# torognes/vsearch

Hardware: AMD Instinct MI355X
Metric: GCUPS (useful DP cells/s of the search16 global-alignment path: DP + traceback + CIGAR) (higher is better)
Workload: dtype int16

## Files before the change

vsearch_amd/csrc/vsx_device.hip:

```cpp
#include <hip/hip_runtime.h>
#include <type_traits>
#include <cstdlib>
#include <atomic>
#include "vsx_internal.h"

typedef unsigned int u32;
typedef unsigned int u32x4 __attribute__((ext_vector_type(4)));
typedef unsigned int u32x3 __attribute__((ext_vector_type(3)));
typedef short s2 __attribute__((ext_vector_type(2)));
typedef unsigned short us2 __attribute__((ext_vector_type(2)));

#define DEV __device__ __forceinline__
struct __attribute__((aligned(4))) Pair2 { unsigned int x, y; };

#define SIGN2 0x80008000u

DEV s2 S2(u32 x) { return __builtin_bit_cast(s2, x); }
DEV us2 U2(u32 x) { return __builtin_bit_cast(us2, x); }
DEV u32 UI(s2 x) { return __builtin_bit_cast(u32, x); }
DEV u32 UI(us2 x) { return __builtin_bit_cast(u32, x); }

DEV u32 sadd(u32 a, u32 b) { return UI(__builtin_elementwise_add_sat(S2(a), S2(b))); }
DEV u32 ssub(u32 a, u32 b) { return UI(__builtin_elementwise_sub_sat(S2(a), S2(b))); }
DEV u32 pmax(u32 a, u32 b) { return UI(__builtin_elementwise_max(S2(a), S2(b))); }
// ... 911 lines not shown
              u32 cv = vin((u32) (uint16_t) P.hleft[ii < 0 ? 0 : ii]);
              if (TOPPAD && L == 0 && xs < pad) cv = vin((u32) (uint16_t) (((xs == pad - 1) ? 0 : -P.top_open) + (xs - pad - 1) * tl));
              tbL[64 + tid] = cv;
            }
        }
      else if (L == 0)
        {
#pragma unroll
          for (int cc = 0; cc < 17; ++cc)
            {
              int c = c0 - 1 + cc;
              if (c > jj) c = jj;
              const u32 corner = (u32) (uint16_t) (((TOPPAD && pad > 0) ? -P.top_open : 0) - (pad + 2) * tl);
              tbL[(cc + 1) * 64 + tid] = (c < 0) ? vin(corner) : vin((u32) (uint16_t) (P.htop[c] - pad * tl));
            }
        }
      else
        {
          const int Lp = L - 1;
          const int sp = Lp >> 4, lp = Lp & 15;
          stage_top(rowck + (size_t) VSX_CK_SLOT(CK8, g, lp) * (CK8 ? 3 : 4), VSX_ROWCK_PAIR_DW(CK8), (long) ((size_t) sp * steps) + (long) (c0 - 1 + lp),
                    (long) (rowsteps >> 1) - 1);
          if (c0 == 0) tbL[64 + tid] = vin((u32) (uint16_t) P.hleft[i0 - 1]);
        }
      stage_symbols(c0);

      u32 hp[RT], ee[RT], qa[RT];
      const u32 qrq_i = pen_pk(P.qrq_i_pk);
      const u32 rq_i = pen_pk(P.rq_i_pk);
      const bool lastrow_here = lastpos && (!MID || hh == 1);
      const u32 qrq_last = lastrow_here ? pen_pk(P.qrq_r_pk) : qrq_i;
      const u32 rq_last = lastrow_here ? pen_pk(P.rq_r_pk) : rq_i;
      if (m == 0)
        {
#pragma unroll
          for (int x = 0; x < RT; ++x)
            {
              int ii = i0 + r0h + x; if (ii > Q - 1) ii = Q - 1;
              if (ii < 0) ii = 0;
              const u32 hl = vin((u32) (uint16_t) P.hleft[ii]);
              hp[x] = hl;
              ee[x] = A::sub(hl, (ii < Q - 1) ? qrq_i : pen_pk(P.qrq_r_pk));
            }
          if (TOPPAD && L == 0 && pad > 0)
            {
#pragma unroll
              for (int x = 0; x < RT; ++x)
                if (r0h + x < pad)
                  {
                    const int xs = r0h + x;
                    const int sh = (xs - pad - 1) * tl;
                    hp[x] = vin((u32) (uint16_t) (((xs == pad - 1) ? 0 : -P.top_open) + sh));
                    ee[x] = A::sub(vin((u32) (uint16_t) (-P.top_open - P.top_step + sh)), qrq_i);
                  }
            }
        }
      else
        {
          if (CK8)
            {
              constexpr int NBQ = MID ? VSX_COLCK_NBH(RT) : VSX_COLCK_NB(R, true);
              Quad fq[NBQ];
              if (MID)
                {
                  const u32 * cb = colck + ((size_t) s * nblk + (size_t) (m - 1)) * COL_DW + VSX_COLCK_CDW(VSX_COLCK_NB(R, true), VSX_CK_SLOT(true, g, l), 0)
                                   + (size_t) (hh * NBQ) * (4 * VSX_COLCK_CG);
#pragma unroll
                  for (int b = 0; b < NBQ; ++b) fq[b] = *reinterpret_cast<const Quad *>(cb + (size_t) b * (4 * VSX_COLCK_CG));
                }
              else
                {
                  const u32 * cb = colck + ((size_t) s * nblk + (size_t) (m - 1)) * COL_DW + VSX_COLCK_CDW(VSX_COLCK_NB(R, true), VSX_CK_SLOT(true, g, l), 0);
#pragma unroll
                  for (int b = 0; b < NBQ; ++b) fq[b] = *reinterpret_cast<const Quad *>(cb + (size_t) b * (4 * VSX_COLCK_CG));
                }
              auto flat = [&](int z) -> u32 {
                const Quad & qd = fq[z >> 2];
                return (z & 3) == 0 ? qd.x : (z & 3) == 1 ? qd.y : (z & 3) == 2 ? qd.z : qd.w;
              };
#pragma unroll
              for (int x = 0; x < RT; ++x)
                {
                  const u32 h = half_lo(flat(x), hi) & 0xffffu;
                  const u32 dd = flat(RT + (x >> 1)) >> (8 * ((x & 1) * 2 + (hi ? 1 : 0)));
                  hp[x] = h;
                  ee[x] = h - (u32) (int) (int8_t) (dd & 0xffu);
                }
            }
          else if (R % 2 == 0)
            {
              const u32 * cb = colck + ((size_t) s * nblk + (size_t) (m - 1)) * COL_DW + VSX_COLCK_DW(R, g * 16 + l, 0);
              constexpr int NBQ = (2 * R) / 4 ? (2 * R) / 4 : 1;
              Quad fq[NBQ];
#pragma unroll
              for (int b = 0; b < NBQ; ++b) fq[b] = *reinterpret_cast<const Quad *>(cb + (size_t) b * (4 * VSX_COLCK_G));
              auto flat = [&](int z) -> u32 {
                const Quad & qd = fq[z >> 2];
                return (z & 3) == 0 ? qd.x : (z & 3) == 1 ? qd.y : (z & 3) == 2 ? qd.z : qd.w;
              };
#pragma unroll
              for (int x = 0; x < R; ++x) { hp[x] = inck(half_lo(flat(x), hi)); ee[x] = inck(half_lo(flat(R + x), hi)); }
            }
          else
            {
#pragma unroll
              for (int x = 0; x < R; ++x)
                {
                  hp[x] = inck(half_lo(colck_at(s, m - 1, g * 16 + l, x), hi));
                  ee[x] = inck(half_lo(colck_at(s, m - 1, g * 16 + l, R + x), hi));
                }
            }
        }
      {
        u32 w[(RT + 3) / 4];
#pragma unroll
        for (int e = 0; e < (RT + 3) / 4; ++e) w[e] = *reinterpret_cast<const u32_unaligned *>(q + i0 + r0h + 4 * e);
#pragma unroll
        for (int x = 0; x < RT; ++x)
          qa[x] = (w[x >> 2] >> (8 * (x & 3))) & 15u;
        if (TOPPAD && L == 0)
          {
#pragma unroll
            for (int x = 0; x < RT; ++x)
              if (r0h + x < pad) qa[x] = 16u;
          }
      }
      u32 diag = tbL[64 + tid] & 0xffffu;

      const bool tile_int = CK8 && RT > 1 && RT <= 16 && !__any(busy && (c0 + cmax >= D - 1));
      const bool top_is_border = (L == 0) && (hh == 0);
      for (int cc = 0; cc <= cmax; ++cc)
        {
          const int c = c0 + cc;
          const u32 qrt = (c < D - 1) ? qrt_i16 : qrt_r16;
          const u32 rt = (c < D - 1) ? rt_i16 : rt_r16;
          const u32 tbv = tbL[(cc + 2) * 64 + tid];
          const u32 topH = tbv & 0xffffu;
          u32 F = top_is_border ? A::sub(topH, qrt) : (tbv >> 16);
          const u32 b16 = (((u32) symL[(cc >> 1) * 64 + tid] >> (4 * (cc & 1))) & 15u) * 32u;
          u32 Hd = diag;
          u32 acc = 0;
          auto row = [&](int x, auto int_tag) __attribute__((always_inline)) {
            constexpr bool INT = decltype(int_tag)::value;
            const u32 V = A::score((int16_t) Ssh[b16 + qa[x]]);
            const u32 h0 = A::add(Hd, V);
            const u32 dU = A::dif(h0, F);
            const u32 h1 = A::max(h0, F);
            const u32 dL = A::dif(h1, ee[x]);
            const u32 h2 = A::max(h1, ee[x]);
            Hd = hp[x];
            hp[x] = h2;
            const bool plain = INT && x < RT - 1;
            const u32 qrq = (x == RT - 1) ? qrq_last : qrq_i;
            const u32 rq = (x == RT - 1) ? rq_last : rq_i;
            const u32 hf = A::sub(h2, qrt);
            const u32 f = INT ? F : A::sub(F, rt);
            const u32 dEU = A::dif(hf, f);
            F = A::max(f, hf);
            const u32 he = plain ? hf : A::sub(h2, qrq);
            const u32 e = plain ? ee[x] : A::sub(ee[x], rq);
            const u32 dEL = A::dif(he, e);
            ee[x] = A::max(e, he);
            acc = A::fun(A::fun(A::fun(A::fun(acc, dU), dL), dEU), dEL);
          };
          if (one_row)
            {
              row(0, std::false_type {});
              bitsL[(cc * ND) * 64 + tid] = (uint16_t) A::one_row_word(acc);
            }
          else
            {
#pragma unroll
              for (int x4 = 0; x4 < RT; x4 += 4)
                if (x4 <= rmax)
                  {
                    if (tile_int)
                      {
#pragma unroll
                        for (int y = 0; y < 4; ++y)
                          if (x4 + y < RT) row(x4 + y, std::true_type {});
                      }
                    else
                      {
#pragma unroll
                        for (int y = 0; y < 4; ++y)
                          if (x4 + y < RT) row(x4 + y, std::false_type {});
                      }
                    bitsL[(cc * ND + (x4 >> 2)) * 64 + tid] = (uint16_t) acc;
                  }
            }
          diag = topH;
        }

      if (busy)
        {
          while (r >= r0h && j >= c0 && (!TOPPAD || i >= 0))
            {
              const int cw = j - c0;
              const int rv = r - r0h;
              const u32 w = bitsL[(cw * ND + (rv >> 2)) * 64 + tid];
              int rid = RT - 4 * (rv >> 2);
              if (rid > 4) rid = 4;
              const u32 bts = A::nibble(w, rid, rv & 3);
              ++al;
              if (op == 1 && (bts & A::EXT_LEFT)) { --j; push(1); }
              else if (op == 2 && (bts & A::EXT_UP)) { --i; --r; push(2); }
              else if (bts & A::LEFT) { if (op != 1) ++ga; --j; push(1); }
              else if (bts & A::UP) { if (op != 2) ++ga; --i; --r; push(2); }
              else { --i; --r; --j; push(0); }
#if VSX_TB_STATS
              atomicAdd(&vsx_tb_stats_dev[3], 1ull);
#endif
            }
          if (r < 0 && L > 0) { --L; r = (L == 0 ? rtop0 : R) - 1; }
        }
    }
#if VSX_TB_STATS
  if (valid) atomicAdd(&vsx_tb_stats_dev[5], 1ull);
#endif
  if (!valid) return;

  VsxPairOut o;
  o.pad = 0; o.nruns = 0; o.run_off = 0;
  if (so.overflow)
    {
      o.score = 32767; o.aligned = 0; o.matches = 0; o.mismatches = 0; o.gaps = 0;
      out[pair_ids[k]] = o;
      rank_note(FL, pair_ids[k], 0u, 32767, 0.0);
      return;
    }
  if (i >= 0) { al += (u32) (i + 1); if (op != 2) ++ga; push_n(2, (u32) (i + 1)); }
  if (j >= 0) { al += (u32) (j + 1); if (op != 1) ++ga; push_n(1, (u32) (j + 1)); }
  if (op >= 0) my[nruns++] = (runlen << 2) | (u32) op;

  u32 ma = 0, mi = 0;
  {
    int qi = Q - 1, tj = D - 1;
    for (u32 x = 0; x < nruns; ++x)
      {
        const u32 w = my[x];
        const int len = (int) (w >> 2);
        const u32 o2 = w & 3u;
        if (o2 == 0)
          {
            for (int b = 0; b < len; b += 8)
              {
                const int rem = (len - b < 8) ? len - b : 8;
                const unsigned long long aw = *reinterpret_cast<const u64_unaligned *>(q + (qi - b - 7));
                const unsigned long long cw = *reinterpret_cast<const u64_unaligned *>(d + (tj - b - 7));
                const unsigned long long ones = 0x0101010101010101ull;
                const unsigned long long x = aw & cw;
                unsigned long long t = (x | (x >> 1) | (x >> 2) | (x >> 3)) & ones;
                if (P.n_mismatch)
                  {
                    const unsigned long long a15 = aw & (aw >> 1) & (aw >> 2) & (aw >> 3);
                    const unsigned long long c15 = cw & (cw >> 1) & (cw >> 2) & (cw >> 3);
                    t &= ~(a15 | c15);
                  }
                t &= ~0ull << (8 * (8 - rem));
                const u32 m8 = (u32) __builtin_popcountll(t);
                ma += m8;
                mi += (u32) rem - m8;
              }
            qi -= len; tj -= len;
          }
        else if (o2 == 1) tj -= len;
        else qi -= len;
      }
  }

  u32 verdict = 0;
  double idv = 0.0;
  if (FL.enabled && nruns > 0) verdict = accept_verdict(FL, Q, D, (int) al, (int) ma, (int) mi, (int) ga, my[nruns - 1], my[0], &idv);
  if (verdict == 3u) nruns = 0;
  rank_note(FL, pair_ids[k], verdict, (int) so.score, idv);

  const unsigned long long base = atomicAdd(cursor, (unsigned long long) nruns);
  if (base + nruns <= runs_capacity)
    for (u32 x = 0; x < nruns; ++x) runs[base + x] = my[x];

  o.score = so.score;
  o.aligned = (uint16_t) al; o.matches = (uint16_t) ma; o.mismatches = (uint16_t) mi; o.gaps = (uint16_t) ga;
  o.pad = (uint16_t) verdict;
  o.nruns = nruns;
  o.run_off = base;
  out[pair_ids[k]] = o;
}


DEV u32 pk_add(u32 a, u32 b) { return UI((us2) (U2(a) + U2(b))); }
DEV u32 pk_sub(u32 a, u32 b) { return psubw(a, b); }
#ifdef VSX_TB2_WAVES_N
#define VSX_TB2_WAVES(R_, MID_) VSX_TB2_WAVES_N
#endif
#ifndef VSX_TB2_WAVES
#define VSX_TB2_WAVES(R_, MID_) 3
#endif
#ifndef VSX_TB_LDSSTAGE
#define VSX_TB_LDSSTAGE 1
#endif
#ifndef VSX_TB_LDSSTAGE_FOR
#define VSX_TB_LDSSTAGE_FOR(R_) ((R_) == 14 || (R_) == 16 || (R_) >= 26)
#endif
template <int R, bool MID>
__global__ void __launch_bounds__(64) __attribute__((amdgpu_waves_per_eu(VSX_TB2_WAVES(R, MID), 8)))
vsx_traceback_tilt_kernel(const VsxDevParams P, const VsxFilterDev FL, const VsxTask * __restrict__ tasks,
                          const u32 * __restrict__ pair_slot, const u32 * __restrict__ pair_ids, u32 npairs,
                          const uint8_t * __restrict__ qc, const uint8_t * __restrict__ tc,
                          const u32 * __restrict__ ck, const VsxSlotOut * __restrict__ slot,
                          u32 * __restrict__ slab, const uint64_t * __restrict__ slab_off,
                          u32 * __restrict__ runs, uint64_t runs_capacity, unsigned long long * cursor,
                          VsxPairOut * __restrict__ out)
{
  static_assert(R >= 4 && (!MID || R % 2 == 0), "R = 1 keeps the first kernel");
  constexpr int RT = MID ? R / 2 : R;
  constexpr int HR = (RT + 1) / 2;
  constexpr int NG = (HR + 3) / 4;
  constexpr int XL = RT - 1 - HR;
  constexpr int NBQ = MID ? VSX_COLCK_NBH(RT) : VSX_COLCK_NB(R, true);
  __shared__ uint8_t Ssh[512];
  __shared__ u32 Ssh4[16];
  constexpr int BITS_DW = 17 * NG * 64, SYM_DW = 10 * 64 / 4;
  __shared__ __attribute__((aligned(16))) u32 arenaL[BITS_DW + SYM_DW + 19 * 64];
  u32 * const bitsL = arenaL;
  uint8_t * const symL = reinterpret_cast<uint8_t *>(arenaL + BITS_DW);
  u32 * const tbL = arenaL + BITS_DW + SYM_DW;
  constexpr bool LSTAGE = (VSX_TB_LDSSTAGE != 0) && VSX_TB_LDSSTAGE_FOR(R) && (BITS_DW + SYM_DW >= 9 * 64 * 4);
  const int tid = (int) threadIdx.x;
  for (int x = tid; x < 512; x += 64)
    Ssh[x] = (uint8_t) (((x & 31) < 16) ? P.matrix[(x >> 5) * 16 + (x & 15)] : (int16_t) (-P.top_step + 2 * P.tilt));
  if (tid < 16)
    {
      const int16_t * mr = P.matrix + tid * 16;
      Ssh4[tid] = (u32) (uint8_t) mr[1] | ((u32) (uint8_t) mr[2] << 8) | ((u32) (uint8_t) mr[4] << 16) | ((u32) (uint8_t) mr[8] << 24);
    }
  __syncthreads();

  const u32 k = blockIdx.x * 64 + (u32) threadIdx.x;
  const bool valid = k < npairs;
  const u32 ts = pair_slot[valid ? k : 0];
  const u32 task = ts >> 3, sl = ts & 7;
  const VsxTask & T = tasks[task];
  const VsxSlotOut so = slot[ts];
  const bool live = valid && !so.overflow;

  const int Q = (int) T.qlen;
  const int D = (int) T.tlen[sl];
  const u32 steps32 = T.steps;
  const unsigned long long dir_off = T.dir_off;
  constexpr size_t COL_DW = (size_t) 64 * 4 * VSX_COLCK_NB(R, true);
  const int g = (int) (sl >> 1) + (int) T.group0;
  const bool hi = (sl & 1) != 0;
  const u32 half_sel = hi ? 0x07060302u : 0x05040100u;
  const u32 bias = P.max3 ? 0x3E00u : 0x8000u;
  const u32 bias_pk = bias * 0x10001u;
  const int tl = P.tilt;
  auto pk16 = [](int v) -> u32 { const u32 x = (u32) v & 0xffffu; return x | (x << 16); };
  auto pk2 = [](int lo, int hi_) -> u32 { return ((u32) lo & 0xffffu) | ((u32) hi_ << 16); };
  const int qrt_i = P.qrt_i, qrt_r = P.qrt_r, rt_i = P.rt_i, rt_r = P.rt_r;
  const int qrq_i = (int) (int16_t) (P.qrq_i_pk & 0xffffu), rq_i = (int) (int16_t) (P.rq_i_pk & 0xffffu);
  const int qrq_r = (int) (int16_t) (P.qrq_r_pk & 0xffffu), rq_r = (int) (int16_t) (P.rq_r_pk & 0xffffu);
  const uint8_t * __restrict__ q = qc + T.qoff;
  const uint8_t * __restrict__ d = tc + T.toff[sl];
  u32 * __restrict__ my = slab + slab_off[valid ? k : 0];

  int i = live ? Q - 1 : -1, j = live ? D - 1 : -1;
  int L = (Q + R - 1) / R - 1;
  int r = R - 1;
  int op = -1;
  u32 runlen = 0, nruns = 0;
  u32 al = 0, ga = 0;
  auto push_n = [&](int newop, u32 n) {
    if (newop == op) { runlen += n; return; }
    if (op >= 0) my[nruns++] = (runlen << 2) | (u32) op;
    op = newop;
    runlen = n;
  };
  auto push = [&](int newop) { push_n(newop, 1u); };

  if (live)
    {
      const int lv = (so.leave == 0xFFFFu) ? -1 : (int) so.leave;
      if (lv < D - 1)
        {
          const u32 n = (u32) (D - 1 - lv);
          al += n; ++ga;
          push_n(1, n);
          j = lv;
        }
    }

  const u32 mA[4] = {0x01010101u, 0x02020202u, 0x04040404u, 0x08080808u};
  const u32 mB[4] = {0x10101010u, 0x20202020u, 0x40404040u, 0x80808080u};

#if VSX_TB_STATS
  const unsigned long long t_kernel0 = __builtin_readcyclecounter();
  unsigned n_iter = 0;
  unsigned long long tphase[6] = {0, 0, 0, 0, 0, 0};
#endif
  for (;;)
    {
      const bool busy = (i >= 0) && (j >= 0);
      if (!__any(busy)) break;
#if VSX_TB_STATS
      ++n_iter;
#endif

      u32 Qb = (u32) Q, stb = steps32;
      unsigned long long dob = dir_off;
      asm volatile("" : "+v"(Qb), "+v"(stb), "+v"(dob));
      const int total_lanes = ((int) Qb + R - 1) / R;
      const int rcnt0 = (int) Qb - (total_lanes - 1) * R;
      const int pad = R - rcnt0;
      const int nstrips = (total_lanes + 15) >> 4;
      const size_t steps = stb;
      const size_t nblk = (steps + 15) >> 4;
      const size_t rowsteps = ((size_t) nstrips * steps + 1) & ~(size_t) 1;
      const size_t rowck_dw = (rowsteps >> 1) * VSX_ROWCK_PAIR_DW(true);
      const u32 * __restrict__ rowck = ck + dob;
      const u32 * __restrict__ colck = rowck + rowck_dw;
      const u32 * __restrict__ midck = colck + (size_t) nstrips * nblk * COL_DW;
      const int s = L >> 4, l = L & 15;
      const int jj = busy ? j : 0;
      const int m = (jj + l) >> 4;
      const int c0 = (16 * m - l) > 0 ? 16 * m - l : 0;
      const int c0b = (m >= 1 && 16 * (m - 1) - l > 0) ? 16 * (m - 1) - l : 0;
      const int i0 = (L == 0) ? -pad : rcnt0 + (L - 1) * R;
      const bool lastpos = (L == total_lanes - 1);
      const int hh = (MID && busy && r >= RT) ? 1 : 0;
      const int r0h = hh * RT;
      const bool lastrow_here = lastpos && (!MID || hh == 1);
      const bool top_is_border = (L == 0) && (hh == 0);
#if VSX_TB_STATS & 1
      {
        const unsigned key = busy ? (((unsigned) task & 0x3FFu) << 22) | ((unsigned) L << 12) | ((unsigned) m << 1) | (unsigned) hh : 0xFFFFFFFFu;
        bool leader = busy;
        for (int o = 1; o < 8; ++o)
          {
            const unsigned other = (unsigned) __shfl((int) key, (tid & ~7) | ((tid - o) & 7), 64);
            if ((tid & 7) >= o && other == key) leader = false;
          }
        const unsigned long long nb = __popcll(__ballot(busy)), nl = __popcll(__ballot(leader));
        if (tid == 0) { atomicAdd(&vsx_tb_stats_dev[1], nb); atomicAdd(&vsx_tb_stats_dev[2], nl); }
      }
#endif

      struct TileIn { Trio v3[LSTAGE ? 1 : 9]; int par; Quad fq[NBQ]; u32 sw[5]; };
      auto load_tile = [&](TileIn & in, const int cst, const int mleft) __attribute__((always_inline)) {
        in.par = 0;
        if (!top_is_border)
          {
            const u32 * base;
            long gstart;
            if (MID && hh == 1)
              {
                base = midck + (size_t) VSX_CK_SLOT(true, g, l) * 3;
                gstart = (long) ((size_t) s * steps) + (long) (cst - 1 + l);
              }
            else
              {
                const int Lp = L - 1, sp = Lp >> 4, lp = Lp & 15;
                base = rowck + (size_t) VSX_CK_SLOT(true, g, lp) * 3;
                gstart = (long) ((size_t) sp * steps) + (long) (cst - 1 + lp);
              }
            const long p0 = gstart >> 1;
            in.par = (int) (gstart - 2 * p0);
            const u32 * bp = base + p0 * (long) VSX_ROWCK_PAIR_DW(true);
            if (LSTAGE)
              {
#pragma unroll
                for (int e = 0; e < 9; ++e)
                  __builtin_amdgcn_global_load_lds((const __attribute__((address_space(1))) void *) (bp + e * VSX_ROWCK_PAIR_DW(true)),
                                                   (__attribute__((address_space(3))) void *) (arenaL + e * 256), 12, 0, 0);
              }
            else
              {
#pragma unroll
            for (int e = 0; e < 9; ++e) in.v3[LSTAGE ? 0 : e] = *reinterpret_cast<const Trio *>(bp + e * VSX_ROWCK_PAIR_DW(true));
              }
          }
        const u32 * cb = colck + ((size_t) s * nblk + (size_t) (mleft > 0 ? mleft : 0)) * COL_DW + VSX_COLCK_CDW(VSX_COLCK_NB(R, true), VSX_CK_SLOT(true, g, l), 0)
                         + (MID ? (size_t) (hh * NBQ) * (4 * VSX_COLCK_CG) : 0);
#pragma unroll
        for (int b = 0; b < NBQ; ++b) in.fq[b] = *reinterpret_cast<const Quad *>(cb + (size_t) b * (4 * VSX_COLCK_CG));
#pragma unroll
        for (int e = 0; e < 5; ++e) in.sw[e] = *reinterpret_cast<const u32_unaligned *>(d + cst + 4 * e);
      };

      u32 qcd[HR], qsel[HR];
      bool plain_acgt = true;
      {
        u32 w[(RT + 3) / 4];
#pragma unroll
        for (int e = 0; e < (RT + 3) / 4; ++e) w[e] = *reinterpret_cast<const u32_unaligned *>(q + i0 + r0h + 4 * e);
        auto code_of = [&](int x) -> u32 {
          const int xx = x < RT ? x : RT - 1;
          u32 c = (w[xx >> 2] >> (8 * (xx & 3))) & 15u;
          if (L == 0 && r0h + xx < pad) c = 16u;
          return c;
        };
#pragma unroll
        for (int x = 0; x < HR; ++x)
          {
            const u32 a = code_of(x), b = code_of(x + HR);
            qcd[x] = a | (b << 16);
            const u32 ia = (a >> 1) - (a >> 3), ib = (b >> 1) - (b >> 3);
            qsel[x] = ia | 0x0C000C00u | ((4u + ib) << 16);
            plain_acgt = plain_acgt && (a == 1 || a == 2 || a == 4 || a == 8) && (b == 1 || b == 2 || b == 4 || b == 8);
          }
      }
      const bool fastV = !__any(busy && !plain_acgt);

      const u32 qrq_pk_i = pk16(qrq_i), rq_pk_i = pk16(rq_i);
      const u32 qrq_pk_x = pk2(qrq_i, lastrow_here ? qrq_r : qrq_i), rq_pk_x = pk2(rq_i, lastrow_here ? rq_r : rq_i);

      auto recompute = [&](const TileIn & in, const bool border_left, const int cst, const int rmax_raw, const int cmax, const bool tile_int)
                       __attribute__((always_inline)) {
        if (top_is_border)
          {
            const u32 corner = (u32) (uint16_t) (((pad > 0) ? -P.top_open : 0) - (pad + 2) * tl);
#pragma unroll
            for (int e = 0; e < 17; ++e)
              {
                int c = cst - 1 + e;
                if (c > jj) c = jj;
                tbL[e * 64 + tid] = (c < 0) ? (corner & 0xffffu) : (u32) (uint16_t) (P.htop[c] - pad * tl);
              }
          }
        else
          {
            u32 * dst = tbL + tid - in.par * 64;
            if (LSTAGE) asm volatile("s_waitcnt vmcnt(0)" ::: "memory");
#pragma unroll
            for (int e = 0; e < 9; ++e)
              {
                Trio raw;
                if (LSTAGE) raw = *reinterpret_cast<const Trio *>(arenaL + e * 256 + tid * 4);
                else raw = in.v3[LSTAGE ? 0 : e];
                const u32 h0 = (half_lo(raw.x, hi) - bias) & 0xffffu, h1 = (half_lo(raw.y, hi) - bias) & 0xffffu;
                const u32 dd = hi ? (raw.z >> 8) : raw.z;
                const int d0 = (int) (int8_t) (dd & 0xffu), d1 = (int) (int8_t) ((dd >> 16) & 0xffu);
                if (e > 0 || in.par == 0) dst[(2 * e) * 64] = h0 | ((h0 - (u32) d0) << 16);
                dst[(2 * e + 1) * 64] = h1 | ((h1 - (u32) d1) << 16);
              }
            if (cst == 0)
              {
                u32 cv;
                if (MID && hh == 1)
                  {
                    const int xs = RT - 1;
                    int ii = i0 + xs; if (ii > Q - 1) ii = Q - 1;
                    cv = (u32) (uint16_t) P.hleft[ii < 0 ? 0 : ii];
                    if (L == 0 && xs < pad) cv = (u32) (uint16_t) (((xs == pad - 1) ? 0 : -P.top_open) + (xs - pad - 1) * tl);
                  }
                else cv = (u32) (uint16_t) P.hleft[i0 - 1];
                tbL[tid] = cv;
              }
          }
#pragma unroll
        for (int c2 = 0; c2 < 10; ++c2)
          {
            const u32 lo = (in.sw[c2 >> 1] >> (16 * (c2 & 1))) & 15u, hi4 = (in.sw[c2 >> 1] >> (16 * (c2 & 1) + 8)) & 15u;
            symL[c2 * 64 + tid] = (uint8_t) (lo | (hi4 << 4));
          }
        u32 hp[HR], ee[HR];
        if (border_left)
          {
#pragma unroll
            for (int x = 0; x < HR; ++x)
              {
                u32 hv[2], ev[2];
#pragma unroll
                for (int hf_ = 0; hf_ < 2; ++hf_)
                  {
                    const int xs = r0h + x + hf_ * HR;
                    int ii = i0 + xs; if (ii > Q - 1) ii = Q - 1;
                    if (ii < 0) ii = 0;
                    asm volatile("" : "+v"(ii));
                    int hl = P.hleft[ii];
                    int e0 = hl - ((ii < Q - 1) ? qrq_i : qrq_r);
                    if (L == 0 && xs < pad)
                      {
                        const int sh = (xs - pad - 1) * tl;
                        hl = ((xs == pad - 1) ? 0 : -P.top_open) + sh;
                        e0 = -P.top_open - P.top_step + sh - qrq_i;
                      }
                    hv[hf_] = (u32) hl & 0xffffu; ev[hf_] = (u32) e0 & 0xffffu;
                  }
                hp[x] = hv[0] | (hv[1] << 16);
                ee[x] = ev[0] | (ev[1] << 16);
              }
          }
        else
          {
            auto flat = [&](int z) -> u32 {
              const Quad & qd = in.fq[z >> 2];
              return (z & 3) == 0 ? qd.x : (z & 3) == 1 ? qd.y : (z & 3) == 2 ? qd.z : qd.w;
            };
#pragma unroll
            for (int x = 0; x < HR; ++x)
              {
                const int xa = x, xb = (x + HR < RT) ? x + HR : RT - 1;
                const u32 h = pk_sub(__builtin_amdgcn_perm(flat(xb), flat(xa), half_sel), bias_pk);
                const int da = (int) (int8_t) ((flat(RT + (xa >> 1)) >> (8 * ((xa & 1) * 2 + (hi ? 1 : 0)))) & 0xffu);
                const int db = (int) (int8_t) ((flat(RT + (xb >> 1)) >> (8 * ((xb & 1) * 2 + (hi ? 1 : 0)))) & 0xffu);
                hp[x] = h;
                ee[x] = pk_sub(h, ((u32) da & 0xffffu) | ((u32) db << 16));
              }
          }
        const int xmax = rmax_raw >= HR ? HR - 1 : rmax_raw;
        u32 tb_prev = tbL[tid];
        u32 Hd_end = 0, F_end = 0;
        u32 cr_prev = 0, qrt_prev = 0, rt_prev = 0;
        auto sym_at = [&](int it) -> u32 { return ((u32) symL[(it >> 1) * 64 + tid] >> (4 * (it & 1))) & 15u; };
        const bool FASTV_any = fastV;
        u32 tbv_n = tbL[64 + tid];
        u32 cr_n = FASTV_any ? Ssh4[sym_at(0)] : sym_at(0) * 32u;
        u32 sy_n = sym_at(1);
        auto column = [&](const int it, auto int_tag, auto fast_tag, auto first_tag) __attribute__((always_inline)) {
          constexpr bool INT = decltype(int_tag)::value;
          constexpr bool FASTV = decltype(fast_tag)::value;
          constexpr bool FIRST = decltype(first_tag)::value;
          const int c = cst + it;
          const u32 tbv = tbv_n;
          const u32 cr = cr_n;
          cr_n = FASTV ? Ssh4[sy_n] : sy_n * 32u;
          tbv_n = tbL[(it + 2) * 64 + tid];
          sy_n = sym_at(it + 2);
          u32 qrt_pk = 0, rt_pk = 0;
          if (!INT)
            {
              const u32 ql = (u32) ((c < D - 1) ? qrt_i : qrt_r) & 0xffffu, rl = (u32) ((c < D - 1) ? rt_i : rt_r) & 0xffffu;
              qrt_pk = ql | (qrt_prev << 16); rt_pk = rl | (rt_prev << 16);
              qrt_prev = ql; rt_prev = rl;
            }
          else qrt_pk = pk16(qrt_i);
          u32 Hd = __builtin_amdgcn_perm(Hd_end, tb_prev, 0x05040100u);
          u32 F = __builtin_amdgcn_perm(F_end, tbv, 0x05040302u);
          if (top_is_border)
            F = __builtin_amdgcn_perm(F_end, ((tbv & 0xffffu) - (INT ? (u32) qrt_i : (qrt_pk & 0xffffu))), 0x05040100u);
#pragma unroll
          for (int g4 = 0; g4 < NG; ++g4)
            if (4 * g4 <= xmax)
              {
                u32 acc = 0;
#pragma unroll
                for (int x = 4 * g4; x < 4 * g4 + 4; ++x)
                  if (x < HR)
                    {
                      u32 V;
                      if (FASTV) V = __builtin_amdgcn_perm(cr_prev, cr, qsel[x]);
                      else
                        {
                          u32 qc2 = qcd[x];
                          asm volatile("" : "+v"(qc2));
                          V = (u32) Ssh[cr + (qc2 & 0xffffu)] | ((u32) Ssh[cr_prev + (qc2 >> 16)] << 16);
                        }
                      const u32 h0 = pk_add(Hd, V);
                      const u32 dU = ssub(h0, F);
                      const u32 h1 = pmax(h0, F);
                      const u32 dL = ssub(h1, ee[x]);
                      const u32 h2 = pmax(h1, ee[x]);
                      Hd = hp[x];
                      hp[x] = FIRST ? bfi(0x0000FFFFu, h2, hp[x]) : h2;
                      const u32 hf = pk_sub(h2, qrt_pk);
                      const u32 f = INT ? F : pk_sub(F, rt_pk);
                      const u32 dEU = ssub(hf, f);
                      F = pmax(f, hf);
                      const bool plain = INT && x != XL;
                      const u32 he = plain ? hf : pk_sub(h2, x == XL ? qrq_pk_x : qrq_pk_i);
                      const u32 e = plain ? ee[x] : pk_sub(ee[x], x == XL ? rq_pk_x : rq_pk_i);
                      const u32 dEL = ssub(he, e);
                      const u32 en = pmax(e, he);
                      ee[x] = FIRST ? bfi(0x0000FFFFu, en, ee[x]) : en;
                      acc = a_bfi(mA[x & 3], __builtin_amdgcn_perm(dL, dU, 0x0B0A0908u), acc);
                      acc = a_bfi(mB[x & 3], __builtin_amdgcn_perm(dEL, dEU, 0x0B0A0908u), acc);
                    }
                bitsL[(it * NG + g4) * 64 + tid] = acc;
              }
          Hd_end = Hd;
          F_end = F;
          tb_prev = tbv;
          cr_prev = cr;
        };
        auto sweep = [&](auto int_tag, auto fast_tag) __attribute__((always_inline)) {
          column(0, int_tag, fast_tag, std::true_type {});
          for (int it = 1; it <= cmax + 1; ++it) column(it, int_tag, fast_tag, std::false_type {});
        };
        if (tile_int) { if (fastV) sweep(std::true_type {}, std::true_type {}); else sweep(std::true_type {}, std::false_type {}); }
        else          { if (fastV) sweep(std::false_type {}, std::true_type {}); else sweep(std::false_type {}, std::false_type {}); }
      };
      auto walk = [&](const int cst) __attribute__((always_inline)) {
        while (r >= r0h && j >= cst && i >= 0)
          {
            const int cw = j - cst;
            const int rv = r - r0h;
            const bool up_half = rv >= HR;
            const int rx = up_half ? rv - HR : rv;
            const u32 w = bitsL[((cw + (up_half ? 1 : 0)) * NG + (rx >> 2)) * 64 + tid] >> ((rx & 3) + (up_half ? 8 : 0));
            ++al;
            const u32 inI = (op == 1) ? 1u : 0u, inD = (op == 2) ? 1u : 0u;
            const u32 c1 = inI & (w >> 20);
            const u32 c2 = (c1 ^ 1u) & inD & (w >> 4);
            const u32 c12 = c1 | c2;
            const u32 c3 = (c12 ^ 1u) & (w >> 16);
            const u32 c4 = ((c12 | c3) ^ 1u) & w;
            const u32 isI = (c1 | c3) & 1u, isD = (c2 | c4) & 1u;
            const int newop = (int) (isI + 2u * isD);
            ga += ((c3 & (inI ^ 1u)) | (c4 & (inD ^ 1u))) & 1u;
            j -= (int) (isD ^ 1u);
            const int di = (int) (isI ^ 1u);
            i -= di; r -= di;
            if (newop != op)
              {
                if (op >= 0) my[nruns++] = (runlen << 2) | (u32) op;
                op = newop;
                runlen = 0;
              }
            ++runlen;
#if VSX_TB_STATS & 1
            atomicAdd(&vsx_tb_stats_dev[3], 1ull);
#endif
          }
      };

#if VSX_TB_STATS & 2
#define TBMARK(k_) do { __builtin_amdgcn_s_waitcnt(0); const unsigned long long now_ = __builtin_readcyclecounter(); tphase[k_] += now_ - tmark; tmark = now_; } while (0)
      unsigned long long tmark = __builtin_readcyclecounter();
#else
#define TBMARK(k_) do { } while (0)
#endif
#pragma unroll 1
      for (int tno = 0; tno < 2; ++tno)
        {
          const bool need = (tno == 0) ? busy : (busy && (m >= 1) && (r >= r0h) && (i >= 0) && (j >= 0) && (j < c0));
          if (tno == 1 && !__any(need)) break;
          const int cst = tno ? c0b : c0;
          TileIn in;
          load_tile(in, cst, tno ? m - 2 : m - 1);
          TBMARK(3 * tno);
          const int rmax_raw = __builtin_amdgcn_readfirstlane(wave_max_i32(need ? r - r0h : 0));
          const int cmax = __builtin_amdgcn_readfirstlane(wave_max_i32(need ? j - cst : 0));
          const bool tile_int = tno ? true : !__any(busy && (c0 + cmax >= D - 1));
          recompute(in, tno ? (m <= 1) : (m == 0), cst, rmax_raw, cmax, tile_int);
          TBMARK(3 * tno + 1);
          if (need) walk(cst);
          TBMARK(3 * tno + 2);
        }
      if (busy && r < 0 && L > 0) { --L; r = R - 1; }
    }
#if VSX_TB_STATS
  if (valid) atomicAdd(&vsx_tb_stats_dev[5], 1ull);
  if (tid == 0)
    {
      atomicAdd(&vsx_tb_stats_dev[15], __builtin_readcyclecounter() - t_kernel0); atomicAdd(&vsx_tb_stats_dev[0], (unsigned long long) n_iter);
      for (int k2 = 0; k2 < 6; ++k2) atomicAdd(&vsx_tb_stats_dev[8 + k2], tphase[k2]);
    }
#endif
  if (!valid) return;

  VsxPairOut o;
  o.pad = 0; o.nruns = 0; o.run_off = 0;
  if (so.overflow)
    {
      o.score = 32767; o.aligned = 0; o.matches = 0; o.mismatches = 0; o.gaps = 0;
      out[pair_ids[k]] = o;
      rank_note(FL, pair_ids[k], 0u, 32767, 0.0);
      return;
    }
  if (i >= 0) { al += (u32) (i + 1); if (op != 2) ++ga; push_n(2, (u32) (i + 1)); }
  if (j >= 0) { al += (u32) (j + 1); if (op != 1) ++ga; push_n(1, (u32) (j + 1)); }
  if (op >= 0) my[nruns++] = (runlen << 2) | (u32) op;

  u32 ma = 0, mi = 0;
  {
    int qi = Q - 1, tj = D - 1;
    for (u32 x = 0; x < nruns; ++x)
      {
        const u32 w = my[x];
        const int len = (int) (w >> 2);
        const u32 o2 = w & 3u;
        if (o2 == 0)
          {
            for (int b = 0; b < len; b += 8)
              {
                const int rem = (len - b < 8) ? len - b : 8;
                const unsigned long long aw = *reinterpret_cast<const u64_unaligned *>(q + (qi - b - 7));
                const unsigned long long cw = *reinterpret_cast<const u64_unaligned *>(d + (tj - b - 7));
                const unsigned long long ones = 0x0101010101010101ull;
                const unsigned long long x2 = aw & cw;
                unsigned long long t = (x2 | (x2 >> 1) | (x2 >> 2) | (x2 >> 3)) & ones;
                if (P.n_mismatch)
                  {
                    const unsigned long long a15 = aw & (aw >> 1) & (aw >> 2) & (aw >> 3);
                    const unsigned long long c15 = cw & (cw >> 1) & (cw >> 2) & (cw >> 3);
                    t &= ~(a15 | c15);
                  }
                t &= ~0ull << (8 * (8 - rem));
                const u32 m8 = (u32) __builtin_popcountll(t);
                ma += m8;
                mi += (u32) rem - m8;
              }
            qi -= len; tj -= len;
          }
        else if (o2 == 1) tj -= len;
        else qi -= len;
      }
  }

  u32 verdict = 0;
  double idv = 0.0;
  if (FL.enabled && nruns > 0) verdict = accept_verdict(FL, Q, D, (int) al, (int) ma, (int) mi, (int) ga, my[nruns - 1], my[0], &idv);
  if (verdict == 3u) nruns = 0;
  rank_note(FL, pair_ids[k], verdict, (int) so.score, idv);

  const unsigned long long base = atomicAdd(cursor, (unsigned long long) nruns);
  if (base + nruns <= runs_capacity)
    for (u32 x = 0; x < nruns; ++x) runs[base + x] = my[x];

  o.score = so.score;
  o.aligned = (uint16_t) al; o.matches = (uint16_t) ma; o.mismatches = (uint16_t) mi; o.gaps = (uint16_t) ga;
  o.pad = (uint16_t) verdict;
  o.nruns = nruns;
  o.run_off = base;
  out[pair_ids[k]] = o;
}

DEV u32 map4(u32 ch)
{
  const u32 c = ch | 0x20u;
  if (((ch | 0x20u) < 'a') || ((ch | 0x20u) > 'z') || ((ch & 0xC0u) != 0x40u)) return 0;
  switch (c)
    {
    case 'a': return 1;  case 'b': return 14; case 'c': return 2;  case 'd': return 13;
    case 'g': return 4;  case 'h': return 11; case 'k': return 12; case 'm': return 3;
    case 'n': return 15; case 'r': return 5;  case 's': return 6;  case 't': return 8;
    case 'u': return 8;  case 'v': return 7;  case 'w': return 9;  case 'y': return 10;
    default: return 0;
    }
}

__global__ void __launch_bounds__(256)
vsx_encode_kernel(const uint8_t * __restrict__ ascii, uint8_t * __restrict__ codes, uint64_t nbytes)
{
  __shared__ uint8_t lut[256];
  lut[threadIdx.x] = (uint8_t) map4(threadIdx.x);
  __syncthreads();
  const uint64_t nvec = nbytes >> 4;
  const uint64_t stride = (uint64_t) gridDim.x * blockDim.x;
  for (uint64_t v = (uint64_t) blockIdx.x * blockDim.x + threadIdx.x; v < nvec; v += stride)
    {
      const uint4 in = reinterpret_cast<const uint4 *>(ascii)[v];
      u32 w[4] = {in.x, in.y, in.z, in.w};
      u32 o[4];
#pragma unroll
      for (int x = 0; x < 4; ++x)
        o[x] = (u32) lut[w[x] & 0xff] | ((u32) lut[(w[x] >> 8) & 0xff] << 8) |
               ((u32) lut[(w[x] >> 16) & 0xff] << 16) | ((u32) lut[w[x] >> 24] << 24);
      reinterpret_cast<uint4 *>(codes)[v] = make_uint4(o[0], o[1], o[2], o[3]);
    }
  if (blockIdx.x == 0 && threadIdx.x < (nbytes & 15))
    {
      const uint64_t p = (nvec << 4) + threadIdx.x;
      codes[p] = lut[ascii[p]];
    }
}

__global__ void __launch_bounds__(256)
vsx_purity_kernel(const uint8_t * __restrict__ codes, const uint64_t * __restrict__ off,
                  const uint32_t * __restrict__ len, uint64_t nseq, uint8_t * __restrict__ impure)
{
  const uint64_t s = (uint64_t) blockIdx.x * 4 + (threadIdx.x >> 6);
  if (s >= nseq) return;
  const int lane = threadIdx.x & 63;
  const uint8_t * p = codes + off[s];
  const uint32_t n = len[s];
  int bad = 0;
  for (uint32_t x = lane; x < n; x += 64)
    {
      const u32 c = p[x];
      bad |= !((c != 0) && ((c & (c - 1)) == 0));
    }
  const unsigned long long any = __ballot(bad);
  if (lane == 0) impure[s] = any ? 1 : 0;
}

__global__ void __launch_bounds__(256)
vsx_max3_selftest_kernel(u32 * bad)
{
  const u32 x = blockIdx.x * 256u + threadIdx.x;
  if (x > 0x7BFFu) return;
  const u32 edge[8] = {0u, 1u, 0x03FFu, 0x0400u, 0x3C00u, 0x3E00u, 0x7BFEu, 0x7BFFu};
  u32 wrong = 0;
  for (u32 k = 0; k < 64; ++k)
    {
      const u32 h = (x * 2654435761u) ^ (k * 0x9E3779B9u);
      const u32 y = (k < 8) ? edge[k] : (h >> 7) % 0x7C00u;
      const u32 z = (k < 16) ? edge[(k + 3) & 7] : (h >> 17) % 0x7C00u;
      const u32 a = x | (y << 16), b = y | (z << 16), c = z | (x << 16);
      const u32 got = pk_max3_bits(a, b, c);
      const u32 m = x > y ? (x > z ? x : z) : (y > z ? y : z);
      if (got != (m | (m << 16))) ++wrong;
      const u32 pa = h ^ (x << 13), pb = (h * 0x85EBCA6Bu) ^ k;
      const u32 pg = __builtin_amdgcn_perm(pa, pb, 0x0B0A0908u);
      const u32 pe = ((pb >> 15) & 1u) * 0xFFu | (((pb >> 31) & 1u) * 0xFFu) << 8 | (((pa >> 15) & 1u) * 0xFFu) << 16 | (((pa >> 31) & 1u) * 0xFFu) << 24;
      if (pg != pe) atomicAdd(bad + 1, 1u);
    }
  if (wrong) atomicAdd(bad, wrong);
}
static std::atomic<int> g_tb_v1_dev[65];
extern "C" void vsx_internal_set_tb_v2(int device, int on) { g_tb_v1_dev[device < 0 || device > 64 ? 64 : device].store(on ? 0 : 1); }
extern "C" hipError_t vsx_launch_max3_selftest(u32 * d_bad, hipStream_t st)
{
  hipLaunchKernelGGL(vsx_max3_selftest_kernel, dim3((0x7C00 + 255) / 256), dim3(256), 0, st, d_bad);
  return hipGetLastError();
}

static const int kRows[] = {1, 4, 8, 10, 12, 14, 16, 18, 20, 22, 24, 26, 28, 32};

extern "C" const int * vsx_supported_rows(int * count)
{
  *count = (int) (sizeof(kRows) / sizeof(kRows[0]));
  return kRows;
}

extern "C" hipError_t vsx_launch_encode(const uint8_t * d_ascii, uint8_t * d_codes, uint64_t nbytes, hipStream_t st)
{
  if (nbytes == 0) return hipSuccess;
  uint64_t blocks = ((nbytes >> 4) + 255) / 256;
  if (blocks < 1) blocks = 1;
  if (blocks > 256 * 8) blocks = 256 * 8;
  hipLaunchKernelGGL(vsx_encode_kernel, dim3((unsigned) blocks), dim3(256), 0, st, d_ascii, d_codes, nbytes);
  return hipGetLastError();
}

extern "C" hipError_t vsx_launch_purity(const uint8_t * d_codes, const uint64_t * d_off, const uint32_t * d_len,
                                        uint64_t nseq, uint8_t * d_impure, hipStream_t st)
{
  if (nseq == 0) return hipSuccess;
  hipLaunchKernelGGL(vsx_purity_kernel, dim3((unsigned) ((nseq + 3) / 4)), dim3(256), 0, st,
                     d_codes, d_off, d_len, nseq, d_impure);
  return hipGetLastError();
}

#define VSX_FWD_GO(GRID_, ...) hipLaunchKernelGGL((vsx_forward_kernel<__VA_ARGS__>), dim3(GRID_), dim3(64), 0, st, P, d_tasks, q, t, dir, strip, slot, ntasks)
#define VSX_FWD_GO4(GRID_, ...) hipLaunchKernelGGL((vsx_forward_kernel<__VA_ARGS__>), dim3(GRID_), dim3(256), 0, st, P, d_tasks, q, t, dir, strip, slot, ntasks)
template <int R>
static hipError_t launch_fwd2(int track, int nq, int one, const VsxDevParams & P, const VsxTask * d_tasks, uint32_t ntasks,
                              const uint8_t * q, const uint8_t * t, uint32_t * dir, uint2 * strip,
                              VsxSlotOut * slot, hipStream_t st)
{
  if (nq == 8)
    {
      if (!(P.tilt != 0 && !track) || (ntasks & 3u)) return hipErrorInvalidValue;
      if constexpr (R >= 4)
        {
          if (!one) return hipErrorInvalidValue;
          if (P.max3) VSX_FWD_GO4(ntasks / 4, R, false, true, true, 1, true, true); else VSX_FWD_GO4(ntasks / 4, R, false, true, false, 1, true, true);
          return hipGetLastError();
        }
      else return hipErrorInvalidValue;
    }
  if (nq != 1)
    {
      if (!(P.tilt != 0 && !track && (nq == 2 || nq == 4))) return hipErrorInvalidValue;
      if constexpr (R >= 4)
        {
          const uint32_t grid = (ntasks + (uint32_t) nq - 1) / (uint32_t) nq;
          if (nq == 2) { if (P.max3) VSX_FWD_GO(grid, R, false, true, true, 2); else VSX_FWD_GO(grid, R, false, true, false, 2); }
          else         { if (P.max3) VSX_FWD_GO(grid, R, false, true, true, 4); else VSX_FWD_GO(grid, R, false, true, false, 4); }
          return hipGetLastError();
        }
      else return hipErrorInvalidValue;
    }
  if (P.tilt != 0)
    {
      if (track) return hipErrorInvalidValue;
      if constexpr (R >= 4)
        {
          if (one)
            {
              if (P.max3) VSX_FWD_GO(ntasks, R, false, true, true, 1, false, true);
              else VSX_FWD_GO(ntasks, R, false, true, false, 1, false, true);
              return hipGetLastError();
            }
        }
      if (P.max3) VSX_FWD_GO(ntasks, R, false, true, true);
      else VSX_FWD_GO(ntasks, R, false, true);
    }
  else if (track) VSX_FWD_GO(ntasks, R, true);
  else VSX_FWD_GO(ntasks, R, false);
  return hipGetLastError();
}
// ... 79 lines not shown
```

Baseline: 8155.

## Unroll traceback column sweep in blocks with constant LDS offsets and specialized interior path

Restructures the traceback recompute column loop into blocks of 2 or 4 columns (default 4). Each column's LDS offsets and symbol-nibble selection become compile-time constants, and the LDS pointers advance once per block. It adds an all-row-groups specialization for full interior fast tiles, which removes the per-group xmax checks. It also precomputes the top-border F value into the high half of the tbL entries, so the per-column top_is_border branch goes away. The cost is larger code and more register pressure. A new profiling script reports per-loop VALU budgets from the disassembly.

```diff
diff --git a/profiles/tb_budget.py b/profiles/tb_budget.py
--- /dev/null
+++ b/profiles/tb_budget.py
@@ -0,0 +1,146 @@
+#!/usr/bin/env python3
+import argparse
+import collections
+import os
+import re
+import shutil
+import subprocess
+import sys
+import tempfile
+
+sys.path.insert(0, os.path.dirname(os.path.abspath(__file__)))
+from valu_budget import LLVM, ROOT, disasm, extract, is_valu, meta
+
+DEFAULT = ["10,false", "16,false", "20,true", "26,true"]
+
+
+def mangled(args):
+    r, mid = [x.strip() for x in args.split(",")]
+    return ("_Z25vsx_traceback_tilt_kernelILi%sELb%dEEv12VsxDevParams12VsxFilterDevPK7VsxTaskPKjS6_jPKhS8_S6_PK10VsxSlotOutPjPKmSC_mPyP10VsxPairOut"
+            % (r, mid == "true"))
+
+
+def lds_bytes(co, sym):
+    note = subprocess.run([LLVM + "/llvm-readelf", "--notes", co], capture_output=True, text=True).stdout
+    m = re.search(r"\.group_segment_fixed_size:\s*(\d+)(?:(?!\.group_segment_fixed_size)[\s\S])*?\.name:\s*" + re.escape(sym) + r"\n", note)
+    return int(m.group(1)) if m else None
+
+
+def column_loops(ins):
+    idx = {addr: k for k, (addr, _, _, _) in enumerate(ins)}
+    isbr = lambda op: op.startswith("s_branch") or op.startswith("s_cbranch")
+    leaders = {0}
+    for k, (addr, op, _, tgt) in enumerate(ins):
+        if isbr(op) or op == "s_endpgm":
+            if k + 1 < len(ins):
+                leaders.add(k + 1)
+            if tgt in idx:
+                leaders.add(idx[tgt])
+    starts = sorted(leaders)
+    blk = {s: n for n, s in enumerate(starts)}
+    ends = [(starts[n + 1] if n + 1 < len(starts) else len(ins)) - 1 for n in range(len(starts))]
+    succ = [[] for _ in starts]
+    for n, e in enumerate(ends):
+        _, op, _, tgt = ins[e]
+        if isbr(op) and tgt in idx:
+            succ[n].append(blk[idx[tgt]])
+        if not op.startswith("s_branch") and op != "s_endpgm" and n + 1 < len(starts):
+            succ[n].append(n + 1)
+    pred = [[] for _ in starts]
+    for n, ss in enumerate(succ):
+        for t in ss:
+            pred[t].append(n)
+    N = len(starts)
+    full = (1 << N) - 1
+    dom = [full] * N
+    dom[0] = 1
+    changed = True
+    while changed:
+        changed = False
+        for n in range(1, N):
+            d = full
+            for p in pred[n]:
+                d &= dom[p]
+            d |= 1 << n
+            if d != dom[n]:
+                dom[n] = d
+                changed = True
+    loops = {}
+    for t in range(N):
+        for h in succ[t]:
+            if dom[t] >> h & 1:
+                body = loops.setdefault(h, {h})
+                work = [t]
+                while work:
+                    x = work.pop()
+                    if x not in body:
+                        body.add(x)
+                        work.extend(pred[x])
+    has = [any(ins[j][1] == "v_pk_max_i16" for j in range(starts[n], ends[n] + 1)) for n in range(N)]
+    cand = {h: b for h, b in loops.items() if any(has[n] for n in b)}
+    out = []
+    for h, b in sorted(cand.items()):
+        if any(h2 != h and b2 < b for h2, b2 in cand.items()):
+            continue
+        out.append(sorted(j for n in b for j in range(starts[n], ends[n] + 1)))
+    return out
+
+
+def report(lib, args, ops):
+    r, mid = [x.strip() for x in args.split(",")]
+    R, MID = int(r), mid == "true"
+    RT = R // 2 if MID else R
+    HR = (RT + 1) // 2
+    sym = mangled(args)
+    tmp = tempfile.mkdtemp(prefix="vsx_tb_budget_")
+    try:
+        if open(lib, "rb").read(20)[18:20] == b"\xe0\x00":
+            co = lib
+            syms = subprocess.run([LLVM + "/llvm-readelf", "-s", "--wide", co], capture_output=True, text=True).stdout
+        else:
+            co, syms = extract(lib, sym, tmp)
+        md = meta(syms, sym)
+        ins = disasm(co, sym, md["start"])
+        lds = lds_bytes(co, sym)
+    finally:
+        shutil.rmtree(tmp, ignore_errors=True)
+    print("vsx_traceback_tilt_kernel<%s>  (%s): tile of %d rows = %d row pairs" % (args, os.path.relpath(lib, ROOT) if lib.startswith(ROOT) else lib, RT, HR))
+    print("  code %d B, %d instructions, %d VALU;  VGPR %s  SGPR %s  scratch %s B  LDS %s B" % (
+        md["size"], len(ins), sum(is_valu(op) for _, op, _, _ in ins), md["num_vgpr"], md["numbered_sgpr"], md["private_seg_size"], lds))
+    print("  column loops (per column, all row groups live):")
+    print("    %-18s %4s %6s %9s %10s %5s %5s %7s %8s" % ("offsets", "cols", "VALU", "row body", "remainder", "LDS", "SALU", "branch", "scratch"))
+    for members in column_loops(ins):
+        h, e = members[0], members[-1]
+        body = [(ins[j][1], ins[j][2]) for j in members]
+        c = collections.Counter(op for op, _ in body)
+        pairs = c["v_pk_max_i16"] / 4.0
+        cols = pairs / HR
+        fast = c["ds_read_u8"] < pairs
+        valu = sum(n for op, n in c.items() if is_valu(op))
+        perm_row = min(c["v_perm_b32"], int((3 if fast else 2) * pairs))
+        row = sum(n for op, n in c.items() if op.startswith("v_pk_")) + c["v_bfi_b32"] + perm_row
+        rest = collections.Counter({op: n for op, n in c.items() if is_valu(op) and not op.startswith("v_pk_") and op != "v_bfi_b32"})
+        rest["v_perm_b32"] -= perm_row
+        ldsn = sum(n for op, n in c.items() if op.startswith("ds_"))
+        salu = sum(n for op, n in c.items() if op.startswith("s_") and not op.startswith(("s_cbranch", "s_branch", "s_waitcnt", "s_nop")))
+        br = sum(n for op, n in c.items() if op.startswith(("s_cbranch", "s_branch")))
+        scr = sum(n for op, n in c.items() if op.startswith(("scratch_", "buffer_")))
+        print("    +0x%05x..+0x%05x %4.3g %6.1f %9.1f %10.1f %5.1f %5.1f %7.1f %8d   %s score pick, %s tile" % (
+            ins[h][0], ins[e][0], cols, valu / cols, row / cols, (valu - row) / cols, ldsn / cols, salu / cols, br / cols, scr,
+            "fast" if fast else "slow", "interior" if row / pairs < 17.5 - (0 if fast else 1) else "border"))
+        if ops:
+            print("      remainder opcodes per trip: %s" % ", ".join("%s %d" % kv for kv in rest.most_common() if kv[1] > 0))
+
+
+def main():
+    ap = argparse.ArgumentParser()
+    ap.add_argument("--lib", default=os.path.join(ROOT, "vsearch_amd", "libvsx.so"))
+    ap.add_argument("--kernel", action="append", help='template arguments "R,MID" of vsx_traceback_tilt_kernel (repeatable)')
+    ap.add_argument("--ops", action="store_true", help="print the opcode histogram of each loop's remainder too")
+    a = ap.parse_args()
+    for k in a.kernel or DEFAULT:
+        report(a.lib, k, a.ops)
+
+
+if __name__ == "__main__":
+    main()
diff --git a/vsearch_amd/csrc/vsx_device.hip b/vsearch_amd/csrc/vsx_device.hip
--- a/vsearch_amd/csrc/vsx_device.hip
+++ b/vsearch_amd/csrc/vsx_device.hip
@@ -1237,6 +1237,9 @@
 #ifndef VSX_TB_LDSSTAGE_FOR
 #define VSX_TB_LDSSTAGE_FOR(R_) ((R_) == 14 || (R_) == 16 || (R_) >= 26)
 #endif
+#ifndef VSX_TB_COLBLOCK
+#define VSX_TB_COLBLOCK 4
+#endif
 template <int R, bool MID>
 __global__ void __launch_bounds__(64) __attribute__((amdgpu_waves_per_eu(VSX_TB2_WAVES(R, MID), 8)))
 vsx_traceback_tilt_kernel(const VsxDevParams P, const VsxFilterDev FL, const VsxTask * __restrict__ tasks,
@@ -1459,7 +1462,8 @@
               {
                 int c = cst - 1 + e;
                 if (c > jj) c = jj;
-                tbL[e * 64 + tid] = (c < 0) ? (corner & 0xffffu) : (u32) (uint16_t) (P.htop[c] - pad * tl);
+                const u32 hv = (c < 0) ? (corner & 0xffffu) : (u32) (uint16_t) (P.htop[c] - pad * tl);
+                tbL[e * 64 + tid] = hv | ((hv - (u32) ((cst - 1 + e < D - 1) ? qrt_i : qrt_r)) << 16);
               }
           }
         else
@@ -1501,6 +1505,8 @@
         u32 hp[HR], ee[HR];
         if (border_left)
           {
+            int i0b = i0, padb = pad;
+            asm volatile("" : "+v"(i0b), "+v"(padb));
 #pragma unroll
             for (int x = 0; x < HR; ++x)
               {
@@ -1509,15 +1515,15 @@
                 for (int hf_ = 0; hf_ < 2; ++hf_)
                   {
                     const int xs = r0h + x + hf_ * HR;
-                    int ii = i0 + xs; if (ii > Q - 1) ii = Q - 1;
+                    int ii = i0b + xs; if (ii > Q - 1) ii = Q - 1;
                     if (ii < 0) ii = 0;
                     asm volatile("" : "+v"(ii));
                     int hl = P.hleft[ii];
                     int e0 = hl - ((ii < Q - 1) ? qrq_i : qrq_r);
-                    if (L == 0 && xs < pad)
+                    if (L == 0 && xs < padb)
                       {
-                        const int sh = (xs - pad - 1) * tl;
-                        hl = ((xs == pad - 1) ? 0 : -P.top_open) + sh;
+                        const int sh = (xs - padb - 1) * tl;
+                        hl = ((xs == padb - 1) ? 0 : -P.top_open) + sh;
                         e0 = -P.top_open - P.top_step + sh - qrq_i;
                       }
                     hv[hf_] = (u32) hl & 0xffffu; ev[hf_] = (u32) e0 & 0xffffu;
@@ -1547,21 +1553,31 @@
         u32 tb_prev = tbL[tid];
         u32 Hd_end = 0, F_end = 0;
         u32 cr_prev = 0, qrt_prev = 0, rt_prev = 0;
-        auto sym_at = [&](int it) -> u32 { return ((u32) symL[(it >> 1) * 64 + tid] >> (4 * (it & 1))) & 15u; };
-        const bool FASTV_any = fastV;
+        const u32 * tbp = tbL + tid;
+        const uint8_t * syp = symL + tid;
+        u32 * bip = bitsL + tid;
+        auto sym_off = [&](u32 byte, int nib, bool fast) -> u32 {
+          return fast ? ((nib ? byte >> 2 : byte << 2) & 0x3Cu) : ((nib ? byte << 1 : byte << 5) & 0x1E0u);
+        };
+        auto score_ref = [&](u32 byte, int nib, bool fast) -> u32 {
+          const u32 o = sym_off(byte, nib, fast);
+          return fast ? *reinterpret_cast<const u32 *>(reinterpret_cast<const uint8_t *>(Ssh4) + o) : o;
+        };
         u32 tbv_n = tbL[64 + tid];
-        u32 cr_n = FASTV_any ? Ssh4[sym_at(0)] : sym_at(0) * 32u;
-        u32 sy_n = sym_at(1);
-        auto column = [&](const int it, auto int_tag, auto fast_tag, auto first_tag) __attribute__((always_inline)) {
+        u32 cr_n = score_ref(syp[0], 0, fastV);
+        u32 sy_n = syp[0];
+        auto column = [&](const int c, auto k_tag, auto p0_tag, auto int_tag, auto fast_tag, auto allg_tag, auto first_tag) __attribute__((always_inline)) {
+          constexpr int K = decltype(k_tag)::value;
+          constexpr int P0 = decltype(p0_tag)::value;
           constexpr bool INT = decltype(int_tag)::value;
           constexpr bool FASTV = decltype(fast_tag)::value;
+          constexpr bool ALLG = decltype(allg_tag)::value;
           constexpr bool FIRST = decltype(first_tag)::value;
-          const int c = cst + it;
           const u32 tbv = tbv_n;
           const u32 cr = cr_n;
-          cr_n = FASTV ? Ssh4[sy_n] : sy_n * 32u;
-          tbv_n = tbL[(it + 2) * 64 + tid];
-          sy_n = sym_at(it + 2);
+          cr_n = score_ref(sy_n, (K + P0 + 1) & 1, FASTV);
+          tbv_n = tbp[(K + 2) * 64];
+          sy_n = syp[((K + P0 + 2) >> 1) * 64];
           u32 qrt_pk = 0, rt_pk = 0;
           if (!INT)
             {
@@ -1572,11 +1588,9 @@
           else qrt_pk = pk16(qrt_i);
           u32 Hd = __builtin_amdgcn_perm(Hd_end, tb_prev, 0x05040100u);
           u32 F = __builtin_amdgcn_perm(F_end, tbv, 0x05040302u);
-          if (top_is_border)
-            F = __builtin_amdgcn_perm(F_end, ((tbv & 0xffffu) - (INT ? (u32) qrt_i : (qrt_pk & 0xffffu))), 0x05040100u);
 #pragma unroll
           for (int g4 = 0; g4 < NG; ++g4)
-            if (4 * g4 <= xmax)
+            if (g4 == 0 || ALLG || 4 * g4 <= xmax)
               {
                 u32 acc = 0;
 #pragma unroll
@@ -1611,19 +1625,37 @@
                       acc = a_bfi(mA[x & 3], __builtin_amdgcn_perm(dL, dU, 0x0B0A0908u), acc);
                       acc = a_bfi(mB[x & 3], __builtin_amdgcn_perm(dEL, dEU, 0x0B0A0908u), acc);
                     }
-                bitsL[(it * NG + g4) * 64 + tid] = acc;
+                bip[(K * NG + g4) * 64] = acc;
               }
           Hd_end = Hd;
           F_end = F;
           tb_prev = tbv;
           cr_prev = cr;
         };
-        auto sweep = [&](auto int_tag, auto fast_tag) __attribute__((always_inline)) {
-          column(0, int_tag, fast_tag, std::true_type {});
-          for (int it = 1; it <= cmax + 1; ++it) column(it, int_tag, fast_tag, std::false_type {});
+        auto sweep = [&](auto int_tag, auto fast_tag, auto allg_tag) __attribute__((always_inline)) {
+          constexpr int CB = VSX_TB_COLBLOCK;
+          static_assert(CB == 2 || CB == 4, "an even block: the symbol nibble of a column must be a constant");
+          column(cst, std::integral_constant<int, 0> {}, std::integral_constant<int, 0> {}, int_tag, fast_tag, allg_tag, std::true_type {});
+          tbp += 64; bip += NG * 64;
+          int cb = cst + 1;
+          for (int left = cmax + 1; left > 0; left -= CB)
+            {
+              column(cb, std::integral_constant<int, 0> {}, std::integral_constant<int, 1> {}, int_tag, fast_tag, allg_tag, std::false_type {});
+              if (left == 1) break;
+              column(cb + 1, std::integral_constant<int, 1> {}, std::integral_constant<int, 1> {}, int_tag, fast_tag, allg_tag, std::false_type {});
+              if constexpr (CB == 4)
+                {
+                  if (left == 2) break;
+                  column(cb + 2, std::integral_constant<int, 2> {}, std::integral_constant<int, 1> {}, int_tag, fast_tag, allg_tag, std::false_type {});
+                  if (left == 3) break;
+                  column(cb + 3, std::integral_constant<int, 3> {}, std::integral_constant<int, 1> {}, int_tag, fast_tag, allg_tag, std::false_type {});
+                }
+              tbp += CB * 64; syp += (CB / 2) * 64; bip += CB * NG * 64; cb += CB;
+            }
         };
-        if (tile_int) { if (fastV) sweep(std::true_type {}, std::true_type {}); else sweep(std::true_type {}, std::false_type {}); }
-        else          { if (fastV) sweep(std::false_type {}, std::true_type {}); else sweep(std::false_type {}, std::false_type {}); }
+        if (tile_int && fastV && xmax >= 4 * (NG - 1)) sweep(std::true_type {}, std::true_type {}, std::true_type {});
+        else if (tile_int) { if (fastV) sweep(std::true_type {}, std::true_type {}, std::false_type {}); else sweep(std::true_type {}, std::false_type {}, std::false_type {}); }
+        else               { if (fastV) sweep(std::false_type {}, std::true_type {}, std::false_type {}); else sweep(std::false_type {}, std::false_type {}, std::false_type {}); }
       };
       auto walk = [&](const int cst) __attribute__((always_inline)) {
         while (r >= r0h && j >= cst && i >= 0)
```

New measurement: 8297, median of 6. 1.7% higher.
